# zxhuang1698/ZeroShape

Measured on AMD Instinct MI355X. Metric: sdf_query_points_per_sec_vox128, higher is better.
Workload: dtype f16x3

## Files before the change

include/zeroshape_hip.h:

```cpp
#ifndef ZEROSHAPE_HIP_H
#define ZEROSHAPE_HIP_H

#include <stddef.h>
#include <stdint.h>

#ifdef __cplusplus
extern "C" {
#endif

#define ZS_ABI_VERSION 44

int zs_abi_version(void);

const char *zs_last_error(void);


int zs_chamfer_forward(const float *xyz1, const float *xyz2, int b, int n, int m,
                       float *dist1, float *dist2, int *idx1, int *idx2, void *stream);

size_t zs_chamfer_workspace_bytes(int b, int n, int m);
int zs_chamfer_forward_ws(const float *xyz1, const float *xyz2, int b, int n, int m,
                          float *dist1, float *dist2, int *idx1, int *idx2,
                          void *workspace, size_t workspace_bytes, void *stream);

int zs_chamfer_backward(const float *xyz1, const float *xyz2, int b, int n, int m,
// ... 34 lines not shown

int zs_attn_frames(const float *zmean, int batch, int n_cols, const int *frame_col, int n_frames,
                   const float *images, int H, int W, const uint8_t *lut, int R, float *frames, void *stream);

int zs_sdf_split_programs(const void *programs, size_t program_stride_bytes, void *split_programs,
                          size_t split_stride_bytes, int batch, void *stream);
int zs_sdf_query_points_split(const void *split_programs, size_t program_stride_bytes, int batch,
                              const float *points, int m, float *logits, int *tile_flags,
                              void *workspace, void *stream);
int zs_sdf_query_grid_split(const void *split_programs, size_t program_stride_bytes, int batch,
                            const float *axis, int G, int slice_begin, int slice_end,
                            int apply_sigmoid, float *out, int *tile_flags, void *workspace,
                            void *stream);

int zs_sdf_block0_tables(const void *split_programs, size_t program_stride_bytes, int batch, float *tables, void *stream);

int zs_sdf_query_grid_range(const void *programs, size_t program_stride_bytes, int batch,
                            const float *axis, int G, long long point_begin, long long point_end,
                            int apply_sigmoid, float *out, const int *tile_mask, void *workspace,
                            void *stream);
int zs_sdf_query_grid_range_split(const void *split_programs, size_t program_stride_bytes, int batch,
                                  const float *axis, int G, long long point_begin,
                                  long long point_end, int apply_sigmoid, float *out,
                                  int *tile_flags, void *workspace, void *stream);

size_t zs_bf_grid_bytes(void);
size_t zs_bf_scratch_bytes(void);
int zs_bf_lower_bounds(const float *pred, int n, const float *gt_normalized, int m,
                       const float *rotations, int k, float *grid_gt, float *grid_pred,
                       void *scratch, float *lower_bounds, void *stream);
// ... 293 lines not shown
```

zeroshape_amd/_lib.py:

```python
import contextlib
import ctypes
import os

_HERE = os.path.dirname(os.path.abspath(__file__))
LIB_PATH = os.environ.get("ZS_LIB_PATH") or os.path.join(_HERE, "libzeroshape_hip.so")

_c_void_p = ctypes.c_void_p
_c_int = ctypes.c_int
_c_size_t = ctypes.c_size_t
_c_float = ctypes.c_float

class ConvFuse(ctypes.Structure):
    _fields_ = [("in_mode", ctypes.c_int), ("in_tiles", ctypes.c_int), ("in_groups", ctypes.c_int), ("in_gshift", ctypes.c_int),
                ("in_stats", ctypes.c_void_p), ("in_gamma", ctypes.c_void_p), ("in_beta", ctypes.c_void_p),
                ("in_eps", ctypes.c_float), ("out_mode", ctypes.c_int), ("out_groups", ctypes.c_int),
                ("out_stats", ctypes.c_void_p)]


SIGNATURES = {
    "zs_abi_version": (_c_int, []),
    "zs_last_error": (ctypes.c_char_p, []),
    "zs_chamfer_forward": (_c_int, [_c_void_p, _c_void_p, _c_int, _c_int, _c_int,
                                    _c_void_p, _c_void_p, _c_void_p, _c_void_p, _c_void_p]),
    "zs_chamfer_workspace_bytes": (_c_size_t, [_c_int, _c_int, _c_int]),
# ... 14 lines not shown
    "zs_sdf_verdict_stats": (_c_int, [_c_void_p, _c_void_p, _c_int, _c_int, _c_float, _c_float, _c_float, _c_void_p, _c_void_p,
                                      _c_void_p]),
    "zs_sdf_query_points": (_c_int, [_c_void_p, _c_size_t, _c_int, _c_void_p, _c_int,
                                     _c_void_p, _c_void_p, _c_void_p, _c_void_p, _c_void_p]),
    "zs_sdf_query_grid": (_c_int, [_c_void_p, _c_size_t, _c_int, _c_void_p, _c_int, _c_int,
                                   _c_int, _c_int, _c_void_p, _c_void_p, _c_void_p, _c_void_p]),
    "zs_sdf_grid_attn_zmean_scratch_bytes": (_c_size_t, [_c_int, _c_int, _c_int, _c_size_t]),
    "zs_sdf_grid_attn_zmean_chunk": (_c_int, [_c_int, _c_int, _c_int, _c_size_t, ctypes.POINTER(_c_int),
                                              ctypes.POINTER(_c_int)]),
    "zs_sdf_grid_attn_zmean": (_c_int, [_c_void_p, _c_size_t, _c_int, _c_void_p, _c_int, _c_void_p, _c_int, _c_void_p,
                                        _c_void_p, _c_void_p, _c_size_t, _c_void_p]),
    "zs_attn_frames": (_c_int, [_c_void_p, _c_int, _c_int, _c_void_p, _c_int, _c_void_p, _c_int, _c_int, _c_void_p, _c_int,
                                _c_void_p, _c_void_p]),
    "zs_sdf_split_programs": (_c_int, [_c_void_p, _c_size_t, _c_void_p, _c_size_t, _c_int, _c_void_p]),
    "zs_sdf_block0_tables": (_c_int, [_c_void_p, _c_size_t, _c_int, _c_void_p, _c_void_p]),
    "zs_sdf_query_points_split": (_c_int, [_c_void_p, _c_size_t, _c_int, _c_void_p, _c_int,
                                           _c_void_p, _c_void_p, _c_void_p, _c_void_p]),
    "zs_sdf_query_grid_split": (_c_int, [_c_void_p, _c_size_t, _c_int, _c_void_p, _c_int, _c_int,
                                         _c_int, _c_int, _c_void_p, _c_void_p, _c_void_p, _c_void_p]),
    "zs_sdf_query_grid_range": (_c_int, [_c_void_p, _c_size_t, _c_int, _c_void_p, _c_int, ctypes.c_longlong,
                                         ctypes.c_longlong, _c_int, _c_void_p, _c_void_p, _c_void_p, _c_void_p]),
    "zs_sdf_query_grid_range_split": (_c_int, [_c_void_p, _c_size_t, _c_int, _c_void_p, _c_int,
                                               ctypes.c_longlong, ctypes.c_longlong, _c_int, _c_void_p,
                                               _c_void_p, _c_void_p, _c_void_p]),
    "zs_erode_mask": (_c_int, [_c_void_p, _c_int, _c_int, _c_int, _c_int, _c_void_p, _c_void_p]),
    "zs_bf_grid_bytes": (_c_size_t, []),
    "zs_bf_scratch_bytes": (_c_size_t, []),
    "zs_bf_lower_bounds": (_c_int, [_c_void_p, _c_int, _c_void_p, _c_int, _c_void_p, _c_int, _c_void_p,
                                    _c_void_p, _c_void_p, _c_void_p, _c_void_p]),
    "zs_pose_max_batch": (_c_int, []),
# ... 134 lines not shown
    "zs_group_norm_bwd_workspace_bytes": (_c_size_t, [_c_int, _c_int]),
    "zs_group_norm_bwd": (_c_int, [_c_void_p] * 8 + [_c_int, _c_int, _c_int, _c_int, _c_float, _c_void_p, _c_void_p]),
    "zs_max_pool_bwd_nhwc": (_c_int, [_c_void_p] * 3 + [_c_int] * 10 + [_c_void_p]),
    "zs_global_mean_bwd_nhwc": (_c_int, [_c_void_p, _c_void_p, _c_int, _c_int, _c_int, _c_void_p]),
    "zs_upsample2x_bwd_nhwc": (_c_int, [_c_void_p, _c_void_p, _c_int, _c_int, _c_int, _c_int, _c_void_p]),
    "zs_nhwc_to_nchw_masked": (_c_int, [_c_void_p, _c_void_p, _c_void_p, _c_int, _c_int, _c_int, _c_int, _c_void_p]),
    "zs_seen_surface_bwd": (_c_int, [_c_void_p] * 7 + [_c_int, _c_int, _c_int, _c_void_p, _c_void_p, _c_void_p]),
    "zs_intr_param2mtx_bwd": (_c_int, [_c_void_p, _c_void_p, _c_int, _c_int, _c_int, _c_void_p, _c_void_p]),
    "zs_window_tokens_bwd": (_c_int, [_c_void_p] * 5 + [_c_int] * 5 + [_c_void_p]),
    "zs_coord_dsp2_bwd": (_c_int, [_c_void_p] * 4 + [_c_int] * 3 + [_c_void_p]),
    "zs_transform_points": (_c_int, [_c_void_p] * 5 + [_c_int, _c_int, _c_void_p]),
    "zs_resize_bilinear_nhwc": (_c_int, [_c_void_p, _c_void_p] + [_c_int] * 6 + [_c_void_p]),
    "zs_readout_concat_bwd": (_c_int, [_c_void_p, _c_void_p, _c_int, _c_int, _c_int, _c_void_p]),
}

ABI_VERSION = 44
_lib = None


class ZeroShapeHipError(RuntimeError):
    pass


def load():
    global _lib
    if _lib is not None:
        return _lib
    if not os.path.exists(LIB_PATH):
        raise ZeroShapeHipError(
            "HIP library not built: %s is missing (run `python -m zeroshape_amd.build`). "
            "zeroshape_amd has no CPU/PyTorch fallback for this path." % LIB_PATH)
# ... 51 lines not shown
```

zeroshape_amd/csrc/sdf_decoder_split.hip:

```cpp
#include "zs_common.h"
#include <stdlib.h>
#include "sdf_layout.h"
#include "sdf_math.h"
#include "zs_split16.h"
#include "sdf_query.h"
#include "../../include/zeroshape_hip.h"

#include <math.h>
#include <stdint.h>
#include <type_traits>

namespace {

using namespace zs::lay;
using namespace zs::qry;
using zs::dm::gelu_erf;
using zs::dm::softplus100;

typedef float f32x16 __attribute__((ext_vector_type(16)));
typedef float f32x4 __attribute__((ext_vector_type(4)));
typedef float f32x2 __attribute__((ext_vector_type(2)));
typedef unsigned u32x4 __attribute__((ext_vector_type(4)));

constexpr float S_GUARD = 64.0f;
constexpr int KB_U4 = 128;
constexpr int CK = 8;
constexpr int KPW = CK / WAVES;
constexpr int CHUNK_BYTES = CK * KB_U4 * 16;
constexpr int NBUF = 2;
constexpr int KB_TOTAL = G_TOTAL / 2;
constexpr int PRM_WINDOW = 4096;
constexpr int STAGE_FLOATS = NBUF * CHUNK_BYTES / 4;
constexpr int SLAB_TILES = NT - 1;
constexpr int SLAB_U4 = SLAB_TILES * 4 * 64;
constexpr int ZTILES_F4 = NT * 4 * 64;
static_assert(ZSLAB_F4 == 3 * ZTILES_F4, "the workspace slab holds three skip layers' feat partial products");
static_assert(B0_TABLE_FLOATS == PRM_WINDOW, "an image's block-0 tables are loaded as one params window");
constexpr int LDS_FLOATS = PRM_WINDOW + STAGE_FLOATS + WAVES * SLAB_U4 * 4;
static_assert(LDS_FLOATS * 4 == 160 * 1024, "the kernel owns the whole LDS of a CU");
// ... 41 lines not shown
#ifdef ZS_EXP_NO_DMA
    if (gsrc != nullptr) return;
#endif
#ifndef ZS_DMA_MOD
#define ZS_DMA_MOD ""
#endif
    asm volatile("s_mov_b32 m0, %1\n\ts_nop 0\n\tglobal_load_lds_dwordx4 %0, off" ZS_DMA_MOD
                 "\n\tglobal_load_lds_dwordx4 %0, off offset:1024" ZS_DMA_MOD
                 "\n\tglobal_load_lds_dwordx4 %0, off offset:2048" ZS_DMA_MOD
                 "\n\tglobal_load_lds_dwordx4 %0, off offset:3072" ZS_DMA_MOD
                 :
                 : "v"(gsrc), "s"(lds_dst)
                 : "memory");
}

struct AStream {
    const u32x4 *buf[NBUF];
    unsigned dst[NBUF];
    u32x4 hi, lo;
    const char *gsrc;

    DEV void init(const char *prog, u32x4 *stage, unsigned stage_addr, int wave, int lane, int first_byte = 0) {
        const char *g = prog + first_byte + wave * (KPW * KB_U4 * 16) + lane * 16;
        asm volatile("s_waitcnt vmcnt(0) lgkmcnt(0)\n\ts_barrier" ::: "memory");
#pragma unroll
        for (int i = 0; i < NBUF; i++) {
            buf[i] = stage + i * (CK * KB_U4) + lane;
            dst[i] = stage_addr + i * CHUNK_BYTES + wave * (KPW * KB_U4 * 16);
            glds_kblocks(g + i * CHUNK_BYTES, dst[i]);
        }
        gsrc = g + NBUF * CHUNK_BYTES;
        asm volatile("s_waitcnt vmcnt(4)\n\ts_barrier" ::: "memory");
        hi = buf[0][0];
        lo = buf[0][64];
    }
    template <int EXTRA_VM = 0>
    DEV void step(int pos, u32x4 &ahi, u32x4 &alo) {
        ahi = hi;
        alo = lo;
        if (pos == CK - 1) {
            static_assert(EXTRA_VM == 0 || EXTRA_VM == 4, "wait-count variants");
            if (EXTRA_VM == 4)
                asm volatile("s_waitcnt vmcnt(4) lgkmcnt(0)\n\ts_barrier" ::: "memory");
            else
                asm volatile("s_waitcnt vmcnt(0) lgkmcnt(0)\n\ts_barrier" ::: "memory");
            glds_kblocks(gsrc, dst[0]);
            gsrc += CHUNK_BYTES;
            const u32x4 *t = buf[0];
            const unsigned u = dst[0];
            buf[0] = buf[1];
            dst[0] = dst[1];
            buf[1] = t;
            dst[1] = u;
            hi = buf[0][0];
            lo = buf[0][64];
        } else {
#ifndef ZS_EXP_NO_AREAD
            hi = buf[0][(pos + 1) * KB_U4];
            lo = buf[0][(pos + 1) * KB_U4 + 64];
#endif
        }
    }
    DEV void skip(int bytes) { gsrc += bytes; }
    DEV void drain() { asm volatile("s_waitcnt vmcnt(0) lgkmcnt(0)" ::: "memory"); }
};

struct Slab {
    u32x4 *fl;
    PT t7;
    DEV void store(int tile, const PT &p) {
        if (tile == SLAB_TILES) {
            t7 = p;
        } else {
#pragma unroll
            for (int q = 0; q < 4; q++) fl[(tile * 4 + q) * 64] = p.v[q];
        }
// ... 184 lines not shown
DEV void mfma3_cacc(f32x16 &acc, const u32x4 &ahi, const u32x4 &alo, const u32x4 &bhi, const u32x4 &blo, int kb,
                    SIDE &side) {
    asm volatile("s_nop 1\n\tv_mfma_f32_32x32x16_f16 %0, %1, %2, %0" : "+a"(acc) : "v"(alo), "v"(bhi));
    ZS_FENCE;
    side(kb, 0);
    ZS_FENCE;
    asm volatile("s_nop 1\n\tv_mfma_f32_32x32x16_f16 %0, %1, %2, %0" : "+a"(acc) : "v"(ahi), "v"(blo));
    ZS_FENCE;
    side(kb, 1);
    ZS_FENCE;
    asm volatile("s_nop 1\n\tv_mfma_f32_32x32x16_f16 %0, %1, %2, %0" : "+a"(acc) : "v"(ahi), "v"(bhi));
    ZS_FENCE;
    side(kb, 2);
    ZS_FENCE;
}
template <bool YACC = false, typename SIDE = NoSide>
DEV void gemm_one(AStream &s, const PT &X, f32x16 &acc, int pos0, int kb0 = 0, SIDE side = SIDE()) {
#pragma unroll
    for (int j = 0; j < 2; j++) {
        u32x4 ahi, alo;
        s.step((pos0 + j) & (CK - 1), ahi, alo);
        pin(ahi, alo);
        if (YACC)
            mfma3_cacc(acc, ahi, alo, X.v[2 * j], X.v[2 * j + 1], kb0 + j, side);
        else
            mfma3_gaps(acc, ahi, alo, X.v[2 * j], X.v[2 * j + 1], kb0 + j, side);
    }
}
DEV void slab_b(const Slab &sl, int kb, u32x4 &bh, u32x4 &bl) {
    if (kb >= SLAB_TILES * 2) {
        bh = sl.t7.v[(kb & 1) * 2];
        bl = sl.t7.v[(kb & 1) * 2 + 1];
    } else {
        bh = sl.fl[kb * KB_U4];
        bl = sl.fl[kb * KB_U4 + 64];
    }
// ... 170 lines not shown
        rp(prm, b_off, kt, hi, b);
#pragma unroll
        for (int r = 0; r < 16; r++) t[r] = fmaf((x[kt][r] - mean) * rstd, g[r], b[r]);
        sl.store(kt, pack_tile(t));
    }
}

DEV void load_params(float *prm, const float *prog_params, int start, int count) {
    __syncthreads();
    const f32x4 *src = reinterpret_cast<const f32x4 *>(prog_params + start);
    f32x4 *dst = reinterpret_cast<f32x4 *>(prm);
    for (int i = threadIdx.x; i < count / 4; i += WAVES * 64) dst[i] = src[i];
    __syncthreads();
}

template <bool MASK>
DEV void attn_tile(AStream &s, const PT &q, f32x16 &o, float &m_run, float &z_run, float c, int hi,
                   int pos0) {
    f32x16 S = zero16();
    gemm_one(s, q, S, pos0);
    float mt = -INFINITY;
#pragma unroll
    for (int r = 0; r < 16; r++) {
        if (MASK) {
            const int rw = (r & 3) + 8 * (r >> 2) + 4 * hi;
            S[r] = rw < L - 32 * (LT - 1) ? S[r] : -INFINITY;
        }
        mt = fmaxf(mt, S[r]);
    }
    mt *= c;
    constexpr float LAZY = 8.0f;
    if (__builtin_amdgcn_ballot_w64(mt > m_run + LAZY) != 0) {
        mt = half_max(mt);
        const float m_new = fmaxf(m_run, mt);
        const float alpha = __builtin_amdgcn_exp2f(m_run - m_new);
        z_run *= alpha;
#pragma unroll
        for (int r = 0; r < 16; r++) o[r] *= alpha;
        m_run = m_new;
    }
    float zs_ = 0.f;
#pragma unroll
    for (int r = 0; r < 16; r++) {
        const float p = __builtin_amdgcn_exp2f(fmaf(S[r], c, -m_run));
        S[r] = p;
        zs_ += p;
    }
    z_run += zs_;
    gemm_one(s, pack_tile(S), o, pos0 + 2);
}

#ifdef ZS_EXP_TIMING
#define ZS_STAMP(i) do { if (dbg) dbg[i] = __builtin_amdgcn_s_memtime(); } while (0)
#else
#define ZS_STAMP(i) do { } while (0)
#endif
DEV float decode_tile(const char *prog, float *prm, u32x4 *stage, unsigned stage_addr, u32x4 *slab,
                      const float *tbl, float px, float py, float pz, int wave, int lane, float &guard,
                      unsigned long long *dbg) {
    const int hi = lane >> 5;
    const float *prog_params = reinterpret_cast<const float *>(prog) + REC_FLOATS;
    constexpr int QKV_BYTES = 3 * NT * 2 / CK * CHUNK_BYTES;
    static_assert(3 * NT * 2 % CK == 0, "AStream::skip passes whole chunks");
    AStream s;
    s.init(prog, stage, stage_addr, wave, lane, tbl ? QKV_BYTES : 0);
    Slab sl;
    sl.fl = slab;
    ZS_STAMP(0);

    load_params(prm, prog_params, W_PP, 1024);
    f32x16 y[NT];
#pragma unroll
    for (int kt = 0; kt < NT; kt++) y[kt] = xyz_affine(prm, 0, kt, hi, px, py, pz);

    ZS_STAMP(1);

    const float scale = 0.17677669529663688110f;

#pragma unroll 1
    for (int blk = 0; blk < BLOCKS; blk++) {
        const bool tab = blk == 0 && tbl != nullptr;
        float rstd0 = 0.f, xr = 0.f, yr = 0.f, zr = 0.f;
        if (tab) {
            load_params(prm, tbl, 0, PRM_WINDOW);
            float mean;
            ln_stats(y, mean, rstd0);
            xr = px * rstd0;
            yr = py * rstd0;
            zr = pz * rstd0;
        } else {
            load_params(prm, prog_params, W_BLK + blk * P_BLK_STRIDE, P_BLK_STRIDE);
            layer_norm_lds(y, sl, prm, PB_LN1G, PB_LN1B, hi);
        }
        ZS_STAMP(2 + blk * 4);
#pragma unroll
        for (int nt = 0; nt < NT; nt++) y[nt] += rp16(prm, tab ? B0_BPROJ : PB_BPROJ, nt, hi);

        auto head = [&](int hd, auto Ptag) {
            constexpr int P = decltype(Ptag)::value;
            f32x16 q, k, v;
            if (tab) {
                q = block0_qkv(prm, hd * 3 + 0, hi, xr, yr, zr, rstd0);
                k = block0_qkv(prm, hd * 3 + 1, hi, xr, yr, zr, rstd0);
                v = block0_qkv(prm, hd * 3 + 2, hi, xr, yr, zr, rstd0);
            } else {
                q = rp16(prm, PB_BQKV, hd * 3 + 0, hi);
                gemm_lds(s, sl, q, P);
                k = rp16(prm, PB_BQKV, hd * 3 + 1, hi);
                gemm_lds(s, sl, k, P);
                v = rp16(prm, PB_BQKV, hd * 3 + 2, hi);
                gemm_lds(s, sl, v, P);
            }

            const float c = scale * 1.44269504088896340736f;
            float s_self = 0.f;
            float qq = 0.f;
#pragma unroll
            for (int r = 0; r < 16; r++) {
                s_self = fmaf(q[r], k[r], s_self);
                qq = fmaf(q[r], q[r], qq);
            }
            s_self = half_sum(s_self) * c;
            {
                const float km = prog_params[P_KMAX + blk * HEADS + hd] * scale;
                guard = fmaxf(guard, half_sum(qq) * (km * km));
            }
            const PT qp = pack_tile(q);

            float m_run = -INFINITY, z_run = 0.f;
            f32x16 o = zero16();
#pragma unroll 1
            for (int l2 = 0; l2 < (LT - 1) / 2; l2++) {
                attn_tile<false>(s, qp, o, m_run, z_run, c, hi, P);
                attn_tile<false>(s, qp, o, m_run, z_run, c, hi, (P + 4) & (CK - 1));
            }
            attn_tile<true>(s, qp, o, m_run, z_run, c, hi, P);
            {
                const float m_new = fmaxf(m_run, s_self);
                const float alpha = __builtin_amdgcn_exp2f(m_run - m_new);
                const float p_self = __builtin_amdgcn_exp2f(s_self - m_new);
                const float z = fmaf(half_sum(z_run), alpha, p_self);
                const float inv = 1.0f / z;
                const float a_i = alpha * inv, p_i = p_self * inv;
#pragma unroll
                for (int r = 0; r < 16; r++) o[r] = fmaf(p_i, v[r], o[r] * a_i);
            }
            const PT op = pack_tile(o);
            const bool bump = tab && hd + 1 < HEADS;
            if (bump && (P == 4 || wave >= 2)) s.skip(QKV_BYTES);
#pragma unroll
            for (int nt = 0; nt < NT; nt++) {
                if (P == 0 && nt == 2 && bump && wave < 2) s.skip(QKV_BYTES);
                gemm_one(s, op, y[nt], (P + 4 + 2 * nt) & (CK - 1));
            }
        };
        static_assert((LT - 1) % 2 == 0 && (3 * NT * 2 + LT * 4 + NT * 2) % CK == 4, "head = 11.5 chunks");
#pragma unroll 1
        for (int hd = 0; hd < HEADS; hd += 2) {
            head(hd, std::integral_constant<int, 0>());
            head(hd + 1, std::integral_constant<int, 4>());
        }

        ZS_STAMP(3 + blk * 4);
        if (tab) load_params(prm, prog_params, W_BLK, P_BLK_STRIDE);
        layer_norm_lds(y, sl, prm, PB_LN2G, PB_LN2B, hi);
#pragma unroll
        for (int nt = 0; nt < NT; nt++) y[nt] += rp16(prm, PB_B2, nt, hi);
        ZS_STAMP(4 + blk * 4);
        RowInit bi;
        f32x16 hid = rp16(prm, PB_B1, 0, hi);
        bi.start(prm, PB_B1, 1, hi);
        gemm_lds(s, sl, hid, 0, [&](int kb, int g) {
            if (g == 2 && (kb & 3) == 1) bi.step(kb & ~3);
        });
#pragma unroll 1
// ... 177 lines not shown
    out = half_sum(out);
    ZS_STAMP(15);
    return out + prm[P_B8 - W_IB];
}

template <bool GRID>
__global__ __launch_bounds__(WAVES * 64, 1) void sdf_decode_split_kernel(
    const char *__restrict__ programs, size_t program_stride_bytes, int batch,
    const float *__restrict__ points,
    const float *__restrict__ axis,
    int G, long long first_point,
    int m,
    float *__restrict__ out, int apply_sigmoid, f32x4 *__restrict__ workspace,
    int *__restrict__ tile_flags,
    int static_order,
    const float *__restrict__ block0_tables) {
    __shared__ __attribute__((aligned(16))) float lds[LDS_FLOATS];
    float *prm = lds;
    const int lane = threadIdx.x & 63;
    const int wave = __builtin_amdgcn_readfirstlane(threadIdx.x >> 6);
    u32x4 *stage = reinterpret_cast<u32x4 *>(lds + PRM_WINDOW);
    const unsigned stage_addr = __builtin_amdgcn_readfirstlane(
        (unsigned)(uintptr_t)(__attribute__((address_space(3))) float *)(lds + PRM_WINDOW));
    u32x4 *fl = reinterpret_cast<u32x4 *>(lds + PRM_WINDOW + STAGE_FLOATS) + wave * SLAB_U4 + lane;

    const int tiles_per_img = (m + PTS_PER_BLOCK - 1) / PTS_PER_BLOCK;
    const int total = tiles_per_img * batch;
    int *tile_counter = zs::qry::tile_counter(workspace);
    int *tile_slot = tile_counter + 16 + blockIdx.x;
    const int dyn_tiles = total > (int)gridDim.x ? total - (int)gridDim.x : 0;
    for (int tile = blockIdx.x;;) {
// ... 17 lines not shown
            pz = axis[iz];
        } else {
            const float *q = points + ((size_t)img * m + pc) * 3;
            px = q[0];
            py = q[1];
            pz = q[2];
        }
#ifdef ZS_EXP_TIMING
        unsigned long long *dbg = (blockIdx.x == 0 && threadIdx.x == 0 && tile == 0)
            ? timing_stamps(workspace) : nullptr;
#else
        unsigned long long *dbg = nullptr;
#endif
        float guard = 0.f;
        const float *tbl = block0_tables ? block0_tables + (size_t)img * PRM_WINDOW : nullptr;
        float logit = decode_tile(prog, prm, stage, stage_addr, fl, tbl, px, py, pz, wave, lane, guard, dbg);
        if (apply_sigmoid) logit = 1.0f / (1.0f + expf(-logit));
        const unsigned bad = reinterpret_cast<const unsigned *>(prog)[REC_FLOATS + P_FLAG];
        const bool pt_bad = (__builtin_bit_cast(unsigned, px) & 0x7f800000u) == 0x7f800000u ||
                            (__builtin_bit_cast(unsigned, py) & 0x7f800000u) == 0x7f800000u ||
                            (__builtin_bit_cast(unsigned, pz) & 0x7f800000u) == 0x7f800000u;
        if (bad || pt_bad) logit = __builtin_bit_cast(float, 0x7fc00000u);
        if (tile_flags) {
            const bool over = !(__builtin_bit_cast(unsigned, guard) <= __builtin_bit_cast(unsigned, S_GUARD * S_GUARD));
            if (__builtin_amdgcn_ballot_w64(over || bad != 0) != 0 && lane == 0) tile_flags[tile] = 1;
        }
        if (lane < 32 && p < m) out[(size_t)img * m + p] = logit;
      }
        if (static_order) {
            tile += (int)gridDim.x;
            if (tile >= total) break;
// ... 153 lines not shown
    for (int d = 0; d < 5; d++) red[t][d] = acc[d];
    __syncthreads();
    if (t < 32) {
        const int hh = (t >> 2) & 1, r = (t & 3) + 4 * (t >> 3), o = tile * 32 + hh * 16 + r;
        double sum[5] = {0.0, 0.0, 0.0, 0.0, 0.0};
        for (int w = 0; w < B0_THREADS / 64; w++)
#pragma unroll
            for (int d = 0; d < 5; d++) sum[d] += red[w * 64 + t][d] + red[w * 64 + 32 + t][d];
#pragma unroll
        for (int d = 0; d < 4; d++) out[B0_T + o * 4 + d] = (float)sum[d];
        out[B0_C + o] = (float)(sum[4] + (double)par[P_BLK0 + PB_BQKV + o]);
    }
    if (tile < C / 32 && t < 32) out[B0_BPROJ + tile * 32 + t] = par[P_BLK0 + PB_BPROJ + tile * 32 + t];
}

const float *launch_block0_tables(const void *split_programs, size_t program_stride_bytes, int batch, void *workspace,
                                  hipStream_t st) {
    const char *e = getenv("ZS_SPLIT_BLOCK0_GEMM");
    if (e && atoi(e) != 0) return nullptr;
    if (!block0_tables_fit(batch)) return nullptr;
    float *tables = static_cast<float *>(workspace);
    hipLaunchKernelGGL(block0_window_kernel, dim3(HEADS * 3, batch), dim3(B0_THREADS), 0, st,
                       static_cast<const char *>(split_programs), program_stride_bytes, tables);
    return tables;
}

int launch_counter_reset(void *workspace, hipStream_t st) {
    const char *e = getenv("ZS_SPLIT_STATIC_TILES");
    if (e && atoi(e) != 0) return 1;
    (void)hipMemsetAsync(tile_counter(workspace), 0, sizeof(int), st);
    return 0;
}

int launch_decode_split(const char *who, const void *split_programs, size_t program_stride_bytes, int batch, const Query &q,
                        float *out, int *tile_flags, void *workspace, void *stream) {
    if (q.m == 0) return 1;
    hipStream_t st = static_cast<hipStream_t>(stream);
    const int static_order = launch_counter_reset(workspace, st);
    const float *b0_tables = launch_block0_tables(split_programs, program_stride_bytes, batch, workspace, st);
    hipLaunchKernelGGL(q.points ? sdf_decode_split_kernel<false> : sdf_decode_split_kernel<true>,
                       dim3(decode_grid_size(batch, q.m)), dim3(WAVES * 64), 0, st,
                       static_cast<const char *>(split_programs), program_stride_bytes, batch, q.points, q.axis, q.G,
                       q.first_point, q.m, out, q.apply_sigmoid, static_cast<f32x4 *>(workspace), tile_flags, static_order,
                       b0_tables);
    return zs::check_launch(who) ? 1 : 0;
}

}

extern "C" int zs_sdf_split_programs(const void *programs, size_t program_stride_bytes,
                                     void *split_programs, size_t split_stride_bytes, int batch,
                                     void *stream) {
    if (batch < 0 || batch > 65535) {
        zs::set_err("zs_sdf_split_programs: bad batch %d", batch);
        return 0;
    }
    if (batch == 0) return 1;
    if (!check_programs("zs_sdf_split_programs", programs, program_stride_bytes) ||
        !check_programs("zs_sdf_split_programs", split_programs, split_stride_bytes))
// ... 17 lines not shown
extern "C" int zs_sdf_block0_tables(const void *split_programs, size_t program_stride_bytes, int batch, float *tables,
                                    void *stream) {
    if (batch < 0 || batch > 65535) {
        zs::set_err("zs_sdf_block0_tables: bad batch %d", batch);
        return 0;
    }
    if (batch == 0) return 1;
    if (!tables) {
        zs::set_err("zs_sdf_block0_tables: null pointer");
        return 0;
    }
    if (!check_programs("zs_sdf_block0_tables", split_programs, program_stride_bytes)) return 0;
    hipLaunchKernelGGL(block0_window_kernel, dim3(HEADS * 3, batch), dim3(B0_THREADS), 0, static_cast<hipStream_t>(stream),
                       static_cast<const char *>(split_programs), program_stride_bytes, tables);
    return zs::check_launch("zs_sdf_block0_tables") ? 1 : 0;
}

extern "C" int zs_sdf_query_points_split(const void *split_programs, size_t program_stride_bytes,
                                         int batch, const float *points, int m, float *logits,
                                         int *tile_flags, void *workspace, void *stream) {
    static const char who[] = "zs_sdf_query_points_split";
    Query q;
    if (!points_query(who, split_programs, program_stride_bytes, batch, points, m, logits, workspace, q)) return 0;
    return launch_decode_split(who, split_programs, program_stride_bytes, batch, q, logits, tile_flags, workspace, stream);
}

extern "C" int zs_sdf_query_grid_range_split(const void *split_programs, size_t program_stride_bytes,
                                             int batch, const float *axis, int G, long long point_begin,
                                             long long point_end, int apply_sigmoid, float *out,
                                             int *tile_flags, void *workspace, void *stream) {
// ... 21 lines not shown
```

zeroshape_amd/csrc/sdf_query.h:

```cpp
#pragma once
#include "zs_common.h"
#include "sdf_layout.h"

#include <stddef.h>

namespace zs {
namespace qry {

constexpr int WAVES = 4;
constexpr int PTS_PER_WAVE = 32;
constexpr int PTS_PER_BLOCK = WAVES * PTS_PER_WAVE;
constexpr int MAX_WGS = 256;
constexpr int ZSLAB_F4 = 3 * lay::NT * 4 * 64;

inline int decode_grid_size(int batch, int m) {
    const long long tiles = (long long)batch * ((m + PTS_PER_BLOCK - 1) / PTS_PER_BLOCK);
    return (int)(tiles < MAX_WGS ? tiles : MAX_WGS);
}

constexpr size_t SLAB_REGION_BYTES = (size_t)MAX_WGS * WAVES * ZSLAB_F4 * 16;
constexpr size_t TAIL_BYTES = 4096;
constexpr size_t TAIL_STAMPS = 0, TAIL_TILE_COUNTER = 1024;
constexpr size_t WORKSPACE_BYTES = SLAB_REGION_BYTES + TAIL_BYTES;
constexpr int B0_TABLE_FLOATS = 4096;

__host__ __device__ inline char *workspace_tail(void *workspace) { return static_cast<char *>(workspace) + SLAB_REGION_BYTES; }
__host__ __device__ inline unsigned long long *timing_stamps(void *workspace) {
    return reinterpret_cast<unsigned long long *>(workspace_tail(workspace) + TAIL_STAMPS);
}
__host__ __device__ inline int *tile_counter(void *workspace) {
    return reinterpret_cast<int *>(workspace_tail(workspace) + TAIL_TILE_COUNTER);
}
inline bool block0_tables_fit(int batch) { return (size_t)batch * B0_TABLE_FLOATS * sizeof(float) <= SLAB_REGION_BYTES; }

struct Query {
    const float *points;
    const float *axis;
    int G;
    long long first_point;
    int m;
    int apply_sigmoid;
};

inline bool check_programs(const char *who, const void *programs, size_t stride) {
    if (!programs) {
        set_err("%s: null pointer", who);
        return false;
    }
// ... 62 lines not shown
```

zeroshape_amd/program.py:

```python
import numpy as np

C = 256
NT = C // 32
HEADS = 8
HD = 32
L = 197
LT = 7
HID = 1024
HT = HID // 32
BLOCKS = 2
MLP_LAYERS = 9
SKIP_IN = (2, 4, 6)
GROUP_FLOATS = 256
RING = 8

LANE = np.arange(64)
LANE_I = LANE & 31
LANE_HI = LANE >> 5


def row(r, hi):
    return (r & 3) + 8 * (r >> 2) + 4 * hi


# ... 399 lines not shown
            out[B0_T + tile * 128:B0_T + (tile + 1) * 128] = \
                np.stack([_rowparam64(T[rows, i]) for i in range(4)], axis=-1).reshape(-1)
    return out.astype(np.float32)


def _rowparam64(v):
    v = np.asarray(v, np.float64)
    T = v.shape[0] // 32
    idx = (32 * np.arange(T))[:, None, None] + ROW_TABLE[None, :, :]
    return v[idx].reshape(-1)


def split_consumed_kblocks():
    keep = [kb for kb in range(KB_TOTAL) if not (kb < HEADS * KB_HEAD and kb % KB_HEAD < KB_QKV_HEAD)]
    return np.array(keep)
```

Baseline: 78.40 million.

## Precompute block-0 attention logit tables and stream them in place of K GEMMs

Adds a per-image precompute kernel that folds block-0 keys with the affine Q-projection tables into a small logit matrix (5 columns per key) stored as split f16 operands. The decode kernel then computes block-0 attention scores with a single MFMA per tile against a per-point operand built from normalized coordinates and rstd. The AStream DMA schedule follows a per-wave bit plan that stages these smaller table tiles instead of full K blocks. The aim is to cut both the score GEMM work and the K-block bandwidth in block 0. In exchange it adds an extra launch, more workspace and a fixed scale factor that could affect precision.

Measured after the change: 78.15 million. No clear change (-0.3%).

```diff
diff --git a/include/zeroshape_hip.h b/include/zeroshape_hip.h
--- a/include/zeroshape_hip.h
+++ b/include/zeroshape_hip.h
@@ -8,7 +8,7 @@
 extern "C" {
 #endif
 
-#define ZS_ABI_VERSION 44
+#define ZS_ABI_VERSION 45
 
 int zs_abi_version(void);
 
@@ -73,6 +73,9 @@
                             void *stream);
 
 int zs_sdf_block0_tables(const void *split_programs, size_t program_stride_bytes, int batch, float *tables, void *stream);
+
+int zs_sdf_block0_logit_tables(const void *split_programs, size_t program_stride_bytes, int batch, const float *windows,
+                               void *tables, void *stream);
 
 int zs_sdf_query_grid_range(const void *programs, size_t program_stride_bytes, int batch,
                             const float *axis, int G, long long point_begin, long long point_end,
diff --git a/zeroshape_amd/_lib.py b/zeroshape_amd/_lib.py
--- a/zeroshape_amd/_lib.py
+++ b/zeroshape_amd/_lib.py
@@ -52,6 +52,7 @@
                                 _c_void_p, _c_void_p]),
     "zs_sdf_split_programs": (_c_int, [_c_void_p, _c_size_t, _c_void_p, _c_size_t, _c_int, _c_void_p]),
     "zs_sdf_block0_tables": (_c_int, [_c_void_p, _c_size_t, _c_int, _c_void_p, _c_void_p]),
+    "zs_sdf_block0_logit_tables": (_c_int, [_c_void_p, _c_size_t, _c_int, _c_void_p, _c_void_p, _c_void_p]),
     "zs_sdf_query_points_split": (_c_int, [_c_void_p, _c_size_t, _c_int, _c_void_p, _c_int,
                                            _c_void_p, _c_void_p, _c_void_p, _c_void_p]),
     "zs_sdf_query_grid_split": (_c_int, [_c_void_p, _c_size_t, _c_int, _c_void_p, _c_int, _c_int,
@@ -216,7 +217,7 @@
     "zs_readout_concat_bwd": (_c_int, [_c_void_p, _c_void_p, _c_int, _c_int, _c_int, _c_void_p]),
 }
 
-ABI_VERSION = 44
+ABI_VERSION = 45
 _lib = None
 
 
diff --git a/zeroshape_amd/csrc/sdf_decoder_split.hip b/zeroshape_amd/csrc/sdf_decoder_split.hip
--- a/zeroshape_amd/csrc/sdf_decoder_split.hip
+++ b/zeroshape_amd/csrc/sdf_decoder_split.hip
@@ -23,6 +23,7 @@
 typedef unsigned u32x4 __attribute__((ext_vector_type(4)));
 
 constexpr float S_GUARD = 64.0f;
+constexpr float B0L_SCALE = 8.0f;
 constexpr int KB_U4 = 128;
 constexpr int CK = 8;
 constexpr int KPW = CK / WAVES;
@@ -94,27 +95,53 @@
                  : "memory");
 }
 
+DEV void glds_operand(const char *gsrc, unsigned lds_dst) {
+#ifdef ZS_EXP_NO_DMA
+    if (gsrc != nullptr) return;
+#endif
+    asm volatile("s_mov_b32 m0, %1\n\ts_nop 0\n\tglobal_load_lds_dwordx4 %0, off" ZS_DMA_MOD : : "v"(gsrc), "s"(lds_dst) : "memory");
+}
+
 struct AStream {
     const u32x4 *buf[NBUF];
     unsigned dst[NBUF];
     u32x4 hi, lo;
     const char *gsrc;
-
-    DEV void init(const char *prog, u32x4 *stage, unsigned stage_addr, int wave, int lane, int first_byte = 0) {
-        const char *g = prog + first_byte + wave * (KPW * KB_U4 * 16) + lane * 16;
+    unsigned long long plan;
+    const char *tsrc;
+
+    template <bool PLAN>
+    DEV void stage_next(unsigned lds_dst) {
+        if (PLAN && (plan & 1)) {
+            glds_operand(tsrc, lds_dst);
+            tsrc += 2 * B0L_TILE_BYTES;
+        } else {
+            glds_kblocks(gsrc, lds_dst);
+        }
+        if (PLAN) plan >>= 1;
+        gsrc += CHUNK_BYTES;
+    }
+    DEV void init(const char *prog, u32x4 *stage, unsigned stage_addr, int wave, int lane, int first_byte = 0,
+                  unsigned long long plan_ = 0, const char *table = nullptr) {
+        gsrc = prog + first_byte + wave * (KPW * KB_U4 * 16) + lane * 16;
+        plan = plan_;
+        tsrc = table + lane * 16;
+        const bool short_dma = plan != 0;
         asm volatile("s_waitcnt vmcnt(0) lgkmcnt(0)\n\ts_barrier" ::: "memory");
 #pragma unroll
         for (int i = 0; i < NBUF; i++) {
             buf[i] = stage + i * (CK * KB_U4) + lane;
             dst[i] = stage_addr + i * CHUNK_BYTES + wave * (KPW * KB_U4 * 16);
-            glds_kblocks(g + i * CHUNK_BYTES, dst[i]);
-        }
-        gsrc = g + NBUF * CHUNK_BYTES;
-        asm volatile("s_waitcnt vmcnt(4)\n\ts_barrier" ::: "memory");
+            stage_next<true>(dst[i]);
+        }
+        if (short_dma)
+            asm volatile("s_waitcnt vmcnt(1)\n\ts_barrier" ::: "memory");
+        else
+            asm volatile("s_waitcnt vmcnt(4)\n\ts_barrier" ::: "memory");
         hi = buf[0][0];
         lo = buf[0][64];
     }
-    template <int EXTRA_VM = 0>
+    template <int EXTRA_VM = 0, bool PLAN = false>
     DEV void step(int pos, u32x4 &ahi, u32x4 &alo) {
         ahi = hi;
         alo = lo;
@@ -124,8 +151,7 @@
                 asm volatile("s_waitcnt vmcnt(4) lgkmcnt(0)\n\ts_barrier" ::: "memory");
             else
                 asm volatile("s_waitcnt vmcnt(0) lgkmcnt(0)\n\ts_barrier" ::: "memory");
-            glds_kblocks(gsrc, dst[0]);
-            gsrc += CHUNK_BYTES;
+            stage_next<PLAN>(dst[0]);
             const u32x4 *t = buf[0];
             const unsigned u = dst[0];
             buf[0] = buf[1];
@@ -140,6 +166,11 @@
             lo = buf[0][(pos + 1) * KB_U4 + 64];
 #endif
         }
+    }
+    DEV void step_operand(int pos, u32x4 &a) {
+        a = hi;
+        hi = buf[0][(pos + 2) * KB_U4];
+        lo = buf[0][(pos + 2) * KB_U4 + 64];
     }
     DEV void skip(int bytes) { gsrc += bytes; }
     DEV void drain() { asm volatile("s_waitcnt vmcnt(0) lgkmcnt(0)" ::: "memory"); }
@@ -354,12 +385,12 @@
     side(kb, 2);
     ZS_FENCE;
 }
-template <bool YACC = false, typename SIDE = NoSide>
+template <bool YACC = false, typename SIDE = NoSide, bool PLAN = false>
 DEV void gemm_one(AStream &s, const PT &X, f32x16 &acc, int pos0, int kb0 = 0, SIDE side = SIDE()) {
 #pragma unroll
     for (int j = 0; j < 2; j++) {
         u32x4 ahi, alo;
-        s.step((pos0 + j) & (CK - 1), ahi, alo);
+        s.template step<0, PLAN>((pos0 + j) & (CK - 1), ahi, alo);
         pin(ahi, alo);
         if (YACC)
             mfma3_cacc(acc, ahi, alo, X.v[2 * j], X.v[2 * j + 1], kb0 + j, side);
@@ -560,11 +591,19 @@
     __syncthreads();
 }
 
-template <bool MASK>
-DEV void attn_tile(AStream &s, const PT &q, f32x16 &o, float &m_run, float &z_run, float c, int hi,
+template <bool MASK, bool TAB>
+DEV void attn_tile(AStream &s, const PT &q, const u32x4 &bu, f32x16 &o, float &m_run, float &z_run, float c, int hi,
                    int pos0) {
     f32x16 S = zero16();
-    gemm_one(s, q, S, pos0);
+    if (TAB) {
+        c *= 1.0f / B0L_SCALE;
+        u32x4 a;
+        s.step_operand(pos0, a);
+        asm volatile("" : "+v"(a) : : "memory");
+        S = __builtin_amdgcn_mfma_f32_32x32x16_f16(zs::s16::as_h(a), zs::s16::as_h(bu), S, 0, 0, 0);
+    } else {
+        gemm_one<false, NoSide, true>(s, q, S, pos0);
+    }
     float mt = -INFINITY;
 #pragma unroll
     for (int r = 0; r < 16; r++) {
@@ -593,7 +632,33 @@
         zs_ += p;
     }
     z_run += zs_;
-    gemm_one(s, pack_tile(S), o, pos0 + 2);
+    gemm_one<false, NoSide, true>(s, pack_tile(S), o, pos0 + 2);
+}
+template <int P, bool TAB>
+DEV void attn_tiles(AStream &s, const PT &q, const u32x4 &bu, f32x16 &o, float &m_run, float &z_run, float c, int hi) {
+#pragma unroll 1
+    for (int l2 = 0; l2 < (LT - 1) / 2; l2++) {
+        attn_tile<false, TAB>(s, q, bu, o, m_run, z_run, c, hi, P);
+        attn_tile<false, TAB>(s, q, bu, o, m_run, z_run, c, hi, (P + 4) & (CK - 1));
+    }
+    attn_tile<true, TAB>(s, q, bu, o, m_run, z_run, c, hi, P);
+}
+
+constexpr unsigned long long B0L_PAIR_W0 = 0x1CF, B0L_PAIR_W2 = 0x1E7;
+constexpr unsigned long long b0l_plan(unsigned long long pair) { return pair | pair << 11 | pair << 22 | pair << 33; }
+static_assert((B0L_PAIR_W0 & 3) == 3 && (B0L_PAIR_W2 & 3) == 3, "AStream::init: a planned wave's first two stagings are table operands");
+static_assert(HEADS == 8 && LT == 7 && B0L_TILE_BYTES == 64 * 16, "plan: four head pairs of 11 chunks, 14 K pairs each");
+DEV u32x4 block0_u_operand(float xr, float yr, float zr, float rstd, int hi) {
+    unsigned h01, l01, h23, l23;
+    split2(xr, yr, h01, l01);
+    split2(zr, rstd, h23, l23);
+    const unsigned one = 0x3c00u;
+    u32x4 b;
+    b[0] = hi ? l23 >> 16 : h01;
+    b[1] = hi ? h01 : h23;
+    b[2] = hi ? h23 : one | l01 << 16;
+    b[3] = hi ? one : l01 >> 16 | l23 << 16;
+    return b;
 }
 
 #ifdef ZS_EXP_TIMING
@@ -602,14 +667,15 @@
 #define ZS_STAMP(i) do { } while (0)
 #endif
 DEV float decode_tile(const char *prog, float *prm, u32x4 *stage, unsigned stage_addr, u32x4 *slab,
-                      const float *tbl, float px, float py, float pz, int wave, int lane, float &guard,
+                      const float *tbl, const char *ltbl, float px, float py, float pz, int wave, int lane, float &guard,
                       unsigned long long *dbg) {
     const int hi = lane >> 5;
     const float *prog_params = reinterpret_cast<const float *>(prog) + REC_FLOATS;
     constexpr int QKV_BYTES = 3 * NT * 2 / CK * CHUNK_BYTES;
     static_assert(3 * NT * 2 % CK == 0, "AStream::skip passes whole chunks");
     AStream s;
-    s.init(prog, stage, stage_addr, wave, lane, tbl ? QKV_BYTES : 0);
+    const unsigned long long plan = !ltbl ? 0 : wave == 0 ? b0l_plan(B0L_PAIR_W0) : wave == 2 ? b0l_plan(B0L_PAIR_W2) : 0;
+    s.init(prog, stage, stage_addr, wave, lane, tbl ? QKV_BYTES : 0, plan, ltbl ? ltbl + (wave >> 1) * B0L_TILE_BYTES : prog);
     Slab sl;
     sl.fl = slab;
     ZS_STAMP(0);
@@ -626,7 +692,9 @@
 #pragma unroll 1
     for (int blk = 0; blk < BLOCKS; blk++) {
         const bool tab = blk == 0 && tbl != nullptr;
+        const bool stab = tab && ltbl != nullptr;
         float rstd0 = 0.f, xr = 0.f, yr = 0.f, zr = 0.f;
+        u32x4 bu = {0u, 0u, 0u, 0u};
         if (tab) {
             load_params(prm, tbl, 0, PRM_WINDOW);
             float mean;
@@ -634,6 +702,7 @@
             xr = px * rstd0;
             yr = py * rstd0;
             zr = pz * rstd0;
+            if (stab) bu = block0_u_operand(xr, yr, zr, rstd0, hi);
         } else {
             load_params(prm, prog_params, W_BLK + blk * P_BLK_STRIDE, P_BLK_STRIDE);
             layer_norm_lds(y, sl, prm, PB_LN1G, PB_LN1B, hi);
@@ -642,8 +711,9 @@
 #pragma unroll
         for (int nt = 0; nt < NT; nt++) y[nt] += rp16(prm, tab ? B0_BPROJ : PB_BPROJ, nt, hi);
 
-        auto head = [&](int hd, auto Ptag) {
+        auto head = [&](int hd, auto Ptag, auto Ttag) {
             constexpr int P = decltype(Ptag)::value;
+            constexpr bool STAB = decltype(Ttag)::value;
             f32x16 q, k, v;
             if (tab) {
                 q = block0_qkv(prm, hd * 3 + 0, hi, xr, yr, zr, rstd0);
@@ -671,16 +741,14 @@
                 const float km = prog_params[P_KMAX + blk * HEADS + hd] * scale;
                 guard = fmaxf(guard, half_sum(qq) * (km * km));
             }
-            const PT qp = pack_tile(q);
-
             float m_run = -INFINITY, z_run = 0.f;
             f32x16 o = zero16();
-#pragma unroll 1
-            for (int l2 = 0; l2 < (LT - 1) / 2; l2++) {
-                attn_tile<false>(s, qp, o, m_run, z_run, c, hi, P);
-                attn_tile<false>(s, qp, o, m_run, z_run, c, hi, (P + 4) & (CK - 1));
+            if (STAB) {
+                attn_tiles<P, true>(s, PT(), bu, o, m_run, z_run, c, hi);
+            } else {
+                const PT qp = pack_tile(q);
+                attn_tiles<P, false>(s, qp, bu, o, m_run, z_run, c, hi);
             }
-            attn_tile<true>(s, qp, o, m_run, z_run, c, hi, P);
             {
                 const float m_new = fmaxf(m_run, s_self);
                 const float alpha = __builtin_amdgcn_exp2f(m_run - m_new);
@@ -697,14 +765,19 @@
 #pragma unroll
             for (int nt = 0; nt < NT; nt++) {
                 if (P == 0 && nt == 2 && bump && wave < 2) s.skip(QKV_BYTES);
-                gemm_one(s, op, y[nt], (P + 4 + 2 * nt) & (CK - 1));
+                gemm_one<false, NoSide, true>(s, op, y[nt], (P + 4 + 2 * nt) & (CK - 1));
             }
         };
         static_assert((LT - 1) % 2 == 0 && (3 * NT * 2 + LT * 4 + NT * 2) % CK == 4, "head = 11.5 chunks");
 #pragma unroll 1
         for (int hd = 0; hd < HEADS; hd += 2) {
-            head(hd, std::integral_constant<int, 0>());
-            head(hd + 1, std::integral_constant<int, 4>());
+            if (stab) {
+                head(hd, std::integral_constant<int, 0>(), std::true_type());
+                head(hd + 1, std::integral_constant<int, 4>(), std::true_type());
+            } else {
+                head(hd, std::integral_constant<int, 0>(), std::false_type());
+                head(hd + 1, std::integral_constant<int, 4>(), std::false_type());
+            }
         }
 
         ZS_STAMP(3 + blk * 4);
@@ -912,7 +985,8 @@
     float *__restrict__ out, int apply_sigmoid, f32x4 *__restrict__ workspace,
     int *__restrict__ tile_flags,
     int static_order,
-    const float *__restrict__ block0_tables) {
+    const float *__restrict__ block0_tables,
+    const char *__restrict__ block0_logits) {
     __shared__ __attribute__((aligned(16))) float lds[LDS_FLOATS];
     float *prm = lds;
     const int lane = threadIdx.x & 63;
@@ -960,7 +1034,8 @@
 #endif
         float guard = 0.f;
         const float *tbl = block0_tables ? block0_tables + (size_t)img * PRM_WINDOW : nullptr;
-        float logit = decode_tile(prog, prm, stage, stage_addr, fl, tbl, px, py, pz, wave, lane, guard, dbg);
+        const char *ltbl = block0_logits ? block0_logits + (size_t)img * B0L_IMAGE_BYTES : nullptr;
+        float logit = decode_tile(prog, prm, stage, stage_addr, fl, tbl, ltbl, px, py, pz, wave, lane, guard, dbg);
         if (apply_sigmoid) logit = 1.0f / (1.0f + expf(-logit));
         const unsigned bad = reinterpret_cast<const unsigned *>(prog)[REC_FLOATS + P_FLAG];
         const bool pt_bad = (__builtin_bit_cast(unsigned, px) & 0x7f800000u) == 0x7f800000u ||
@@ -1144,6 +1219,55 @@
     if (tile < C / 32 && t < 32) out[B0_BPROJ + tile * 32 + t] = par[P_BLK0 + PB_BPROJ + tile * 32 + t];
 }
 
+__global__ __launch_bounds__(64) void block0_logit_kernel(const char *__restrict__ programs, size_t program_stride_bytes,
+                                                          const float *__restrict__ windows, u32x4 *__restrict__ tables) {
+    __shared__ double red[64][5];
+    const int head = blockIdx.x / LT, lt = blockIdx.x - head * LT, img = blockIdx.y, lane = threadIdx.x, hl = lane >> 5;
+    const u32x4 *kb0 = reinterpret_cast<const u32x4 *>(programs + (size_t)img * program_stride_bytes) +
+                       (size_t)(head * (G_HEAD / 2) + G_QKV_HEAD / 2 + lt * 4) * KB_U4;
+    const float *win = windows + (size_t)img * PRM_WINDOW;
+    const float *T = win + B0_T + 3 * head * 128 + hl * 64, *cq = win + B0_C + 3 * head * 32 + hl * 16;
+    double acc[5] = {0.0, 0.0, 0.0, 0.0, 0.0};
+#pragma unroll
+    for (int j = 0; j < 2; j++) {
+        const u32x4 h4 = kb0[j * KB_U4 + lane], l4 = kb0[j * KB_U4 + 64 + lane];
+#pragma unroll
+        for (int e = 0; e < 8; e++) {
+            const unsigned hw = h4[e >> 1] >> (16 * (e & 1)), lw = l4[e >> 1] >> (16 * (e & 1));
+            const double k = (double)(float)__builtin_bit_cast(_Float16, (unsigned short)hw) +
+                             (double)(float)__builtin_bit_cast(_Float16, (unsigned short)lw);
+            const int r = 8 * j + e;
+#pragma unroll
+            for (int d = 0; d < 4; d++) acc[d] += k * (double)T[r * 4 + d];
+            acc[4] += k * (double)cq[r];
+        }
+    }
+#pragma unroll
+    for (int d = 0; d < 5; d++) red[lane][d] = acc[d];
+    __syncthreads();
+    const int rw = lane & 31;
+    float M[5];
+#pragma unroll
+    for (int d = 0; d < 5; d++) M[d] = 32 * lt + rw < L ? (float)(red[rw][d] + red[rw + 32][d]) * B0L_SCALE : 0.f;
+    unsigned h01, l01, h23, l23, h4, l4;
+    split2(M[0], M[1], h01, l01);
+    split2(M[2], M[3], h23, l23);
+    split2(M[4], 0.f, h4, l4);
+    u32x4 a;
+    if (hl == 0) {
+        a[0] = h01;
+        a[1] = h23;
+        a[2] = (h4 & 0xffffu) | h01 << 16;
+        a[3] = h01 >> 16 | h23 << 16;
+    } else {
+        a[0] = h23 >> 16 | h4 << 16;
+        a[1] = l01;
+        a[2] = l23;
+        a[3] = l4 & 0xffffu;
+    }
+    tables[((size_t)img * (HEADS * LT) + blockIdx.x) * 64 + lane] = a;
+}
+
 const float *launch_block0_tables(const void *split_programs, size_t program_stride_bytes, int batch, void *workspace,
                                   hipStream_t st) {
     const char *e = getenv("ZS_SPLIT_BLOCK0_GEMM");
@@ -1155,6 +1279,19 @@
     return tables;
 }
 
+const char *launch_block0_logits(const void *split_programs, size_t program_stride_bytes, int batch, void *workspace,
+                                 const float *windows, hipStream_t st) {
+    if (!windows) return nullptr;
+    const char *e = getenv("ZS_SPLIT_BLOCK0_S_GEMM");
+    if (e && atoi(e) != 0) return nullptr;
+    if (!block0_logit_tables_fit(batch)) return nullptr;
+    char *tables = block0_logit_tables(workspace, batch);
+    hipLaunchKernelGGL(block0_logit_kernel, dim3(HEADS * LT, batch), dim3(64), 0, st,
+                       static_cast<const char *>(split_programs), program_stride_bytes, windows,
+                       reinterpret_cast<u32x4 *>(tables));
+    return tables;
+}
+
 int launch_counter_reset(void *workspace, hipStream_t st) {
     const char *e = getenv("ZS_SPLIT_STATIC_TILES");
     if (e && atoi(e) != 0) return 1;
@@ -1168,11 +1305,12 @@
     hipStream_t st = static_cast<hipStream_t>(stream);
     const int static_order = launch_counter_reset(workspace, st);
     const float *b0_tables = launch_block0_tables(split_programs, program_stride_bytes, batch, workspace, st);
+    const char *b0_logits = launch_block0_logits(split_programs, program_stride_bytes, batch, workspace, b0_tables, st);
     hipLaunchKernelGGL(q.points ? sdf_decode_split_kernel<false> : sdf_decode_split_kernel<true>,
                        dim3(decode_grid_size(batch, q.m)), dim3(WAVES * 64), 0, st,
                        static_cast<const char *>(split_programs), program_stride_bytes, batch, q.points, q.axis, q.G,
                        q.first_point, q.m, out, q.apply_sigmoid, static_cast<f32x4 *>(workspace), tile_flags, static_order,
-                       b0_tables);
+                       b0_tables, b0_logits);
     return zs::check_launch(who) ? 1 : 0;
 }
 
@@ -1220,6 +1358,23 @@
     hipLaunchKernelGGL(block0_window_kernel, dim3(HEADS * 3, batch), dim3(B0_THREADS), 0, static_cast<hipStream_t>(stream),
                        static_cast<const char *>(split_programs), program_stride_bytes, tables);
     return zs::check_launch("zs_sdf_block0_tables") ? 1 : 0;
+}
+
+extern "C" int zs_sdf_block0_logit_tables(const void *split_programs, size_t program_stride_bytes, int batch,
+                                          const float *windows, void *tables, void *stream) {
+    if (batch < 0 || batch > 65535) {
+        zs::set_err("zs_sdf_block0_logit_tables: bad batch %d", batch);
+        return 0;
+    }
+    if (batch == 0) return 1;
+    if (!windows || !tables) {
+        zs::set_err("zs_sdf_block0_logit_tables: null pointer");
+        return 0;
+    }
+    if (!check_programs("zs_sdf_block0_logit_tables", split_programs, program_stride_bytes)) return 0;
+    hipLaunchKernelGGL(block0_logit_kernel, dim3(HEADS * LT, batch), dim3(64), 0, static_cast<hipStream_t>(stream),
+                       static_cast<const char *>(split_programs), program_stride_bytes, windows, static_cast<u32x4 *>(tables));
+    return zs::check_launch("zs_sdf_block0_logit_tables") ? 1 : 0;
 }
 
 extern "C" int zs_sdf_query_points_split(const void *split_programs, size_t program_stride_bytes,
diff --git a/zeroshape_amd/csrc/sdf_query.h b/zeroshape_amd/csrc/sdf_query.h
--- a/zeroshape_amd/csrc/sdf_query.h
+++ b/zeroshape_amd/csrc/sdf_query.h
@@ -32,6 +32,14 @@
     return reinterpret_cast<int *>(workspace_tail(workspace) + TAIL_TILE_COUNTER);
 }
 inline bool block0_tables_fit(int batch) { return (size_t)batch * B0_TABLE_FLOATS * sizeof(float) <= SLAB_REGION_BYTES; }
+constexpr int B0L_TILE_BYTES = 1024;
+constexpr int B0L_IMAGE_BYTES = lay::HEADS * lay::LT * B0L_TILE_BYTES;
+__host__ __device__ inline char *block0_logit_tables(void *workspace, int batch) {
+    return static_cast<char *>(workspace) + (size_t)batch * B0_TABLE_FLOATS * sizeof(float);
+}
+inline bool block0_logit_tables_fit(int batch) {
+    return (size_t)batch * (B0_TABLE_FLOATS * sizeof(float) + B0L_IMAGE_BYTES) <= SLAB_REGION_BYTES;
+}
 
 struct Query {
     const float *points;
diff --git a/zeroshape_amd/program.py b/zeroshape_amd/program.py
--- a/zeroshape_amd/program.py
+++ b/zeroshape_amd/program.py
@@ -437,3 +437,75 @@
 def split_consumed_kblocks():
     keep = [kb for kb in range(KB_TOTAL) if not (kb < HEADS * KB_HEAD and kb % KB_HEAD < KB_QKV_HEAD)]
     return np.array(keep)
+
+
+B0L_TILE_HALVES = 64 * 8
+B0L_SCALE = 8.0
+KB_KV_HEAD = G_KV_HEAD // 2
+
+
+def block0_k(split_prog):
+    words = np.ascontiguousarray(split_prog).view(np.uint32)
+    K = np.zeros((HEADS, LT * 32, HD), np.float64)
+    for h in range(HEADS):
+        for lt in range(LT):
+            for j in range(2):
+                v = _kblock_values(words, h * KB_HEAD + KB_QKV_HEAD + 4 * lt + j)
+                K[h, (32 * lt + LANE_I)[:, None], ROW_TABLE[LANE_HI][:, 8 * j:8 * j + 8]] = v
+    return K
+
+
+def block0_logit_matrix(split_prog):
+    win = block0_window(split_prog).astype(np.float64)
+    K = block0_k(split_prog)
+    M = np.zeros((HEADS, LT * 32, 5), np.float64)
+    for h in range(HEADS):
+        T = _from_rowparam4(win[B0_T + 3 * h * 128:B0_T + (3 * h + 1) * 128])
+        c = _from_rowparam(win[B0_C + 3 * h * 32:B0_C + (3 * h + 1) * 32])
+        M[h] = K[h] @ np.concatenate([T, c[:, None]], axis=1)
+    M[:, L:] = 0.0
+    return M.astype(np.float32)
+
+
+def _from_rowparam4(v):
+    out = np.empty((32, 4), np.asarray(v).dtype)
+    out[ROW_TABLE.reshape(-1)] = np.asarray(v).reshape(32, 4)
+    return out
+
+
+def pack_logit_tables(M):
+    M = np.ascontiguousarray(M, np.float32) * np.float32(B0L_SCALE)
+    hi16, hif = f16_round(M)
+    lo16, _ = f16_round(M - hif)
+    k = np.zeros(M.shape[:2] + (16,), np.uint16)
+    k[..., 0:5], k[..., 5:10], k[..., 10:15] = hi16, hi16, lo16
+    k = k.reshape(HEADS, LT, 32, 2, 8)
+    return np.ascontiguousarray(k.transpose(0, 1, 3, 2, 4)).reshape(HEADS, LT, 64, 8)
+
+
+def unpack_logit_tables(tables):
+    t = np.ascontiguousarray(tables).view(np.float16).reshape(HEADS, LT, 2, 32, 8)
+    k = t.transpose(0, 1, 3, 2, 4).reshape(HEADS, LT * 32, 16).astype(np.float64)
+    return k[..., 0:5], k[..., 5:10], k[..., 10:15], k[..., 15]
+
+
+def block0_logit_tables(split_prog):
+    return pack_logit_tables(block0_logit_matrix(split_prog))
+
+
+def split_logit_schedule():
+    out = []
+    for i, kb in enumerate(split_consumed_kblocks()):
+        chunk, slot = divmod(i, 8)
+        src = ("prog", int(kb))
+        if kb < HEADS * KB_HEAD:
+            h, r = divmod(int(kb), KB_HEAD)
+            r -= KB_QKV_HEAD
+            if 0 <= r < KB_KV_HEAD and r % 4 < 2:
+                src = ("table", h, r // 4) if r % 4 == 0 else ("dead",)
+        out.append((chunk, slot, src))
+    return out
+
+
+def split_logit_consumed_kblocks():
+    return np.array([src[1] for _, _, src in split_logit_schedule() if src[0] == "prog"])
```
